# dylandreimerink/mimic

Hardware: AMD Instinct MI355X
Metric: Mpkts/s (device-resident, one XDP program over 64-1500B batches) (higher is better)
Workload: dtype u64; 1 GPU; cfg2: 1M x 64B xdp_md, 36-slot parse+hash DROP/PASS classifier, per-CPU array E=4 S=8; packets_per_gpu=1048576, vcpus_per_gpu=262144, schedule=interleaved, parallelism=dp1, batches_rotated=8, working_set_bytes=713031680, program_slots=36, engine=spread_own, batches_per_launch=8

## Files before the change

### mimic_amd/csrc/engine.cpp

```cpp
#include <hip/hip_runtime.h>

#include <algorithm>
#include <atomic>
#include <cstdarg>
#include <cstdlib>
#include <cstdio>
#include <cstring>
#include <map>
#include <string>
#include <chrono>
#include <condition_variable>
#include <memory>
#include <mutex>
#include <thread>
#include <unordered_map>
#include <vector>

#include "../../include/mimic_amd.h"
#include "blkcache.h"
#include "layout.h"
#include "hashmap.h"
#include "jit.h"
#include "skb.h"

// ... 1835 lines not shown
            while (q > 1 && (P % q || 256u * q / P > rows)) q--;
            kp->own_q = q;
            own = ko.state > 0 && P % q == 0 && 256u * q / P <= rows && 256u * q / P >= 1u &&
                  mimic_jit_step_bound(ko.info, kp->max_tail_calls) <= kp->budget;
            spread = own;
        }
        if (!own && (knob == 1 || (knob != 0 && (uint64_t)b->n >= 8ull * cpu_lanes))) {
            if ((rc = spread_build(vm, false))) return rc;
            const JitKernel &ks = vm->kern[K_SPREAD];
            spread = ks.state > 0 && mimic_jit_step_bound(ks.info, kp->max_tail_calls) <= kp->budget;
            if (knob != 1 && !ks.info.spread_rows && cpu_lanes > 16384) spread = false;
        }
    }
    const bool cxk = jit && kp->cancel_any;
    if (cxk) {
        spread = own = false;
        if (!vm->kern[K_CX + ctx].state) {
            const std::vector<std::pair<uint32_t, uint32_t>> vc = percpu_slots(vm).vc;
            JitOpts o;
            o.ctx_kind = ctx;
            o.vc_slots = &vc;
            o.no_early_loads = !lane.info.early_loads;
            o.ctx_check = true;
            if ((rc = kern_build(vm, o, "", &vm->kern[K_CX + ctx]))) return rc;
        }
    }
    *out = KernChoice{proc_jit ? K_PROC : own ? K_OWN : spread ? K_SPREAD : cxk ? K_CX + (int)ctx : K_LANE + (int)ctx,
                      jit, spread, own};
    const JitKernel &k = vm->kern[out->form];
    if (proc_jit && (!k.fn || !k.info.proc_ok)) return fail(vm, MIMIC_EDEVICE, "process: no single-process JIT kernel (engine)");
    return 0;
}

static int run_xdp_impl(mimic_vm *vm, uint32_t prog_id, const mimic_xdp_batch *b, const mimic_xdp_results *res,
                        hipStream_t st_in, uint64_t first_index, const SkbRun *skb, const StepRun *step,
                        const CtxRun *cx, ManyRun *mr) {
    if (!vm || !b || !res) return MIMIC_EINVAL;
    if (prog_id >= vm->progs.size()) return fail(vm, MIMIC_EINVAL, "no program with id '%u' is loaded", prog_id);
    if (const int brc = xdp_batch_check(vm, b, -1)) return brc;
    if (skb && b->n > 0 && (!b->pkt_off || !b->pkt_len)) return fail(vm, MIMIC_EINVAL, "missing packet arrays");
    if (cx && cx->all && cx->per_packet) return fail(vm, MIMIC_EINVAL, "one context for the batch or one per packet, not both");
    if (cx && cx->all && !cx->all->pinned) return fail(vm, MIMIC_EDEVICE, "the context was made without a device");
    if (cx && cx->per_packet)
        for (uint32_t i = 0; i < b->n; i++)
            if (cx->per_packet[i] && !cx->per_packet[i]->pinned)
                return fail(vm, MIMIC_EDEVICE, "packet %u: the context was made without a device", i);
    if (!skb) {
        const int rc = skb_settle(vm);
        if (rc) return rc;
    }
    if (!skb && vm->skb_leaked)
        return fail(vm, MIMIC_ENOTSUP, "xdp_md batches after sk_buff batches are not supported (mimic_skb_release first)");
    const uint32_t ctx = skb ? CTX_SKB : CTX_XDP;
    hipSetDevice(vm->s.device);
    int rc = upload_tables(vm);
    if (!rc) rc = flush_host(vm);
    if (rc) return rc;
    hipStream_t st = st_in ? st_in : vm->stream;
    const uint32_t cpu_lanes = step ? 1u : (uint32_t)vm->s.vcpu_count;
    const bool proc_jit = step && step->jit;
    bool extra = false;
    if (!step && b->schedule == MIMIC_SCHED_EXPLICIT && b->cpu)
        for (uint32_t i = 0; i < b->n && !extra; i++) extra = b->cpu[i] == -1 || b->cpu[i] == vm->s.vcpus;
    const uint32_t lanes = cpu_lanes + (extra ? 2u : 0u);
    const uint32_t S = stack_size(vm);
    const PrivPlan pp = priv_plan(vm);
// ... 238 lines not shown
    }
    vm->last_exec = jit ? (own ? MIMIC_EXEC_SPREAD_OWN : spread ? MIMIC_EXEC_SPREAD : MIMIC_EXEC_JIT) : MIMIC_EXEC_INTERP;
    if (jit && ji.defer) {
        if (lanes > vm->defer_cap || !vm->d_defer_any) {
            hipStreamSynchronize(st);
            hipFree(vm->d_defer);
            vm->d_defer = nullptr;
            HIP_OK(vm, hipMalloc(&vm->d_defer, (uint64_t)plan * sizeof(DeferRec)));
            HIP_OK(vm, hipMemset(vm->d_defer, 0, (uint64_t)plan * sizeof(DeferRec)));
            vm->defer_cap = plan;
            if (!vm->d_defer_any) {
                HIP_OK(vm, hipMalloc(&vm->d_defer_any, 64));
                HIP_OK(vm, hipMemset(vm->d_defer_any, 0, 64));
            }
        }
        if (++vm->defer_epoch == 0) vm->defer_epoch = 1;
        kp.defer = vm->d_defer;
        kp.defer_any = vm->d_defer_any;
        kp.defer_epoch = vm->defer_epoch;
    }
    if (jit && ji.hash_combine) vm->comb_used = true;
    if (mr) {
        mr->used = jit && own && !ji.defer && mr->k >= 1 && mr->k <= MIMIC_MANY_MAX;
        if (mr->used) {
            kp.many_n = mr->k;
            for (uint32_t q = 0; q < mr->k; q++) {
                const mimic_xdp_batch &bq = mr->b[q];
                kp.many[q] = BatchRef{bq.pkt_data, bq.pkt_off, bq.pkt_len, mr->r[q].r0, mr->r[q].status, mr->r[q].steps,
                                      mr->r[q].err_pc,
                                      (bq.pkt_off ? 0u : bq.pkt_stride) | (uint64_t)(bq.pkt_len ? 0u : bq.pkt_len_all) << 32};
            }
        }
    }
    if (jit) {
        if (mimic_jit_launch(kern.fn, &kp, st))
            return fail(vm, MIMIC_EDEVICE, "launch: %s", hipGetErrorString(hipGetLastError()));
        if (ji.defer && mimic_launch_xdp_resume(&kp, st))
            return fail(vm, MIMIC_EDEVICE, "launch: %s", hipGetErrorString(hipGetLastError()));
    } else if (step) {
        if (mimic_launch_xdp(&kp, nullptr, st))
            return fail(vm, MIMIC_EDEVICE, "launch: %s", hipGetErrorString(hipGetLastError()));
    } else {
        const KParams *dkp = nullptr;
        const int slot = kp_slot(vm, kp, st, &dkp);
        if (slot < 0) return slot;
        if (mimic_launch_xdp(&kp, dkp, st))
            return fail(vm, MIMIC_EDEVICE, "launch: %s", hipGetErrorString(hipGetLastError()));
        HIP_OK(vm, hipEventRecord(vm->kp_ev[slot], st));
        vm->kp_used[slot] = true;
    }
    if (jit && ji.hash_chunk) {
        for (const HostMap &m : vm->maps) {
            if (!m.chunk) continue;
            const DMap dm = to_dmap(m);
            if (mimic_launch_hash_compact(vm->arena, &dm, st))
                return fail(vm, MIMIC_EDEVICE, "launch: %s", hipGetErrorString(hipGetLastError()));
        }
    }
    if (jit && kp.spread_part) {
        const DMap dm = to_dmap(vm->maps[ji.spread_map]);
        if (mimic_launch_spread_reduce(kp.spread_part, kp.lanes / 256u, kp.cpu_lanes, ji.spread_roww, ji.spread_n,
                                       vm->arena + dm.dev_off + (uint64_t)kp.vcpu_begin * dm.dev_stride, dm.dev_stride, st))
            return fail(vm, MIMIC_EDEVICE, "launch: %s", hipGetErrorString(hipGetLastError()));
    }
    if (kp.cancel_any) {
        auto mark = [&](mimic_ctx *c) -> int {
            std::lock_guard<std::mutex> lk(c->mu);
            std::vector<hipEvent_t> keep;
// ... 935 lines not shown
```

### mimic_amd/csrc/jit.cpp

```cpp
#include <hip/hip_runtime.h>
#include <hip/hiprtc.h>

#include <algorithm>
#include <cinttypes>
#include <cstdarg>
#include <cstdio>
#include <cstring>
#include <cstdlib>
#include <unistd.h>
#include <map>
#include <mutex>
#include <set>
#include <string>
#include <vector>

#include "../../include/mimic_amd.h"
#include "layout.h"
#include "jit.h"

namespace {

#include "jit_headers.inc"

struct Emitter {
// ... 390 lines not shown
        E.line("      srow_ = lam_ >= lam0_ ? lam_ - lam0_ : lam_ + kp.cpu_lanes - lam0_;");
        E.line("      sbase_ = SM_.backing_addr + (uint32_t)L.cpu * SM_.addr_period; }");
        emit_xdp_load();
        emit_process_start("P + L.M + 1", "    uint64_t r10 = kp.static_next + kp.frame_size;");
        emit_entry_dispatch("kp.entry_prog");
        emit_programs();
        emit_result_stores("kq_", nullptr);
        emit_loop_close();
        E.line("#if SPREAD_ROWS");
        E.line("  __syncthreads();");
        E.line("  if (kp.spread_part && kp.cpu_lanes == SPREAD_ROWS) {");
        E.line("    spread_t *pt_ = (spread_t *)kp.spread_part + (size_t)blockIdx.x * (SPREAD_ROWS * SPREAD_ROWW);");
        E.line("    for (uint32_t w_ = threadIdx.x; w_ < SPREAD_ROWS * SPREAD_ROWW; w_ += 256u) {");
        E.line("      const uint32_t r_ = w_ / SPREAD_ROWW, q_ = w_ - r_ * SPREAD_ROWW;");
        E.line("      const uint32_t lr_ = lam0_ + r_ < SPREAD_ROWS ? lam0_ + r_ : lam0_ + r_ - SPREAD_ROWS;");
        E.line("      pt_[lr_ * SPREAD_ROWW + q_] = sacc_[w_];");
        E.line("    }");
        E.line("  } else");
        E.line("  for (uint32_t w_ = threadIdx.x; w_ < SPREAD_ROWS * SPREAD_ROWW; w_ += 256u) {");
        E.line("    const spread_t v_ = sacc_[w_];");
        E.line("    if (!v_) continue;");
        E.line("    const uint32_t r_ = w_ / SPREAD_ROWW, q_ = w_ - r_ * SPREAD_ROWW;");
        E.line("    const uint32_t lr_ = lam0_ + r_ < kp.cpu_lanes ? lam0_ + r_ : lam0_ + r_ - kp.cpu_lanes;");
        E.line("    spread_t *d_ = (spread_t *)(kp.arena + SM_.dev_off + (size_t)(kp.vcpu_begin + lr_) * SM_.dev_stride) + q_;");
        E.line("    __hip_atomic_fetch_add((GAS spread_t *)d_, v_, __ATOMIC_RELAXED, __HIP_MEMORY_SCOPE_AGENT);");
        E.line("  }");
        E.line("#endif");
        emit_kernel_close();
    }

    void emit_owned() {
        emit_kernel_open("0xffffffffu");
        emit_lane_open();
        E.line("  const uint32_t oP_ = kp.per_lane, oQ_ = kp.own_q, oS_ = oP_ / oQ_, oR_ = 256u / oS_;");
        E.line("  const uint32_t orow_ = threadIdx.x %% oR_, oj_ = threadIdx.x / oR_, olane_ = blockIdx.x * oR_ + orow_;");
        E.line("  const uint32_t osh_ = olane_ >= kp.sched_shift ? olane_ - kp.sched_shift : olane_ + kp.cpu_lanes - kp.sched_shift;");
        E.line("#define OWN_IDX_I(k_) ((oj_ < oS_ && olane_ < kp.cpu_lanes && (uint64_t)(oj_ + (k_) * oS_) * kp.cpu_lanes + osh_ < kp.n) ? (uint32_t)((uint64_t)(oj_ + (k_) * oS_) * kp.cpu_lanes + osh_) : NO_PKT)");
        E.line("#define OWN_IDX_C(k_) ((threadIdx.x + 256u * (k_) < oR_ * oP_ && (uint64_t)blockIdx.x * oR_ * oP_ + threadIdx.x + 256u * (k_) < kp.n) ? (uint32_t)((uint64_t)blockIdx.x * oR_ * oP_ + threadIdx.x + 256u * (k_)) : NO_PKT)");
        E.line("#define OWN_IDX(k_) (kp.sched == SCHED_CHUNKED ? OWN_IDX_C(k_) : OWN_IDX_I(k_))");
        E.line("  const uint32_t oi_ = OWN_IDX(0u);");
        E.line("  const bool ochk_ = kp.sched == SCHED_CHUNKED;");
        E.line("  const uint64_t ostr64_ = ochk_ ? 256ull : (uint64_t)oS_ * kp.cpu_lanes;");
        E.line("  const uint64_t oend_ = (uint64_t)blockIdx.x * oR_ * oP_ + (uint32_t)(oR_ * oP_);");
        E.line("  uint32_t ofl_ = __builtin_amdgcn_readfirstlane((kp.headroom_arr || kp.tailroom_arr || kp.ingress_arr || kp.rxq_arr || kp.egress_arr ? 1u : 0u) | (kp.headroom | kp.tailroom ? 2u : 0u));");
        E.line("  uint32_t ocpu_ = kp.vcpu_begin + olane_, oep_ = kp.entry_prog, or10_ = kp.static_next + kp.frame_size;");
        E.line("  uint32_t ostr_ = ostr64_ < 0xffffffffull ? (uint32_t)ostr64_ : 0xffffffffu;");
        E.line("  uint32_t olim_ = ochk_ && oend_ < kp.n ? (uint32_t)oend_ : kp.n;");
        E.line("  asm volatile(\"\" : \"+s\"(ostr_), \"+s\"(olim_), \"+s\"(ofl_), \"+s\"(oep_), \"+s\"(or10_));");
        E.line("  asm volatile(\"\" : \"+v\"(ocpu_));");
        E.line("  uint32_t oin_ = (uint32_t)kp.ingress, orx_ = (uint32_t)kp.rxq, oeg_ = (uint32_t)kp.egress;");
        E.line("  asm volatile(\"\" : \"+s\"(oin_), \"+s\"(orx_), \"+s\"(oeg_));");
        Emitter head;
        std::swap(head, E);
        E.line("  const DMap SM_ = cget(kp.maps, SPREAD_MAP);");
        E.line("  __shared__ spread_t sacc_[SPREAD_ROWS * SPREAD_ROWW];");
        E.line("  for (uint32_t w_ = threadIdx.x; w_ < SPREAD_ROWS * SPREAD_ROWW; w_ += 256u) sacc_[w_] = 0;");
        E.line("  __shared__ BatchRef obr_[MIMIC_MANY_MAX];");
        E.line("  if (threadIdx.x < (kp.many_n ? kp.many_n : 1u)) obr_[threadIdx.x] = kp.many_n ? cget(kp.many, threadIdx.x) : BatchRef{kp.pkt_data, kp.pkt_off, kp.pkt_len, kp.r0, kp.status, kp.steps, kp.err_pc, kp.pkt_stride | (uint64_t)kp.pkt_len_all << 32};");
        E.line("  __syncthreads();");
        E.line("  uint32_t srow_ = orow_, sbase_ = 0;");
        E.line("  const bool ofw_ = threadIdx.x < oR_ * SPREAD_ROWW && blockIdx.x * oR_ + threadIdx.x / SPREAD_ROWW < kp.cpu_lanes;");
        E.line("  GAS spread_t *const ofd_ = (GAS spread_t *)(kp.arena + SM_.dev_off + (size_t)(kp.vcpu_begin + blockIdx.x * oR_ + threadIdx.x / SPREAD_ROWW) * SM_.dev_stride) + threadIdx.x %% SPREAD_ROWW;");
        E.line("  const spread_t ofv_ = ofw_ ? *ofd_ : (spread_t)0;");
        emit_locals();
        if (pf) E.line("  uint64_t noff_ = 0, poff_ = 0; uint32_t nlen_ = 0, plen_ = 0;");
        E.line("  const uint32_t nb_ = kp.many_n ? kp.many_n : 1u;");
        E.line("  bool bpre_ = false;   // this batch's first descriptor came with the previous batch's last packet");
        E.line("  for (uint32_t bt_ = 0; bt_ < nb_; bt_++) {");
        E.line("  const BatchRef br_ = kp.many_n ? cget(kp.many, bt_) : BatchRef{kp.pkt_data, kp.pkt_off, kp.pkt_len, kp.r0, kp.status, kp.steps, kp.err_pc, kp.pkt_stride | (uint64_t)kp.pkt_len_all << 32};");
        E.line("  uint32_t cstr_ = (uint32_t)br_.compact, clen_ = (uint32_t)(br_.compact >> 32);");
        E.line("  asm volatile(\"\" : \"+v\"(cstr_), \"+v\"(clen_));");
        E.line("  ofl_ = (ofl_ & 3u) | (br_.pkt_off ? 0u : 4u) | (br_.pkt_len ? 0u : 8u);");
        if (pf) {
            E.line("  if (oi_ != NO_PKT) {");
            E.line("    if (!bpre_) { pkt_off_pf(!(ofl_ & 4u), br_.pkt_off, oi_, noff_); pkt_len_pf(!(ofl_ & 8u), br_.pkt_len, oi_, nlen_); }");
            E.line("    poff_ = pkt_off_take(!(ofl_ & 4u), noff_, cstr_, oi_); plen_ = pkt_len_take(!(ofl_ & 8u), nlen_, clen_);");
            E.line("  }");
            E.line("  bpre_ = false;");
        }
        E.line("  uint32_t oni_ = oi_;   // the thread's next packet");
        E.line("  for (uint32_t j = 0; j < oQ_; j++) {   // the thread's packets of its lane, in order");
        E.line("    const uint32_t i = oni_;");
        E.line("    if (i == NO_PKT) break;");
        E.line("    oni_ = NO_PKT;");
        E.line("    if (j + 1u < oQ_) { const uint64_t x_ = (uint64_t)i + ostr_; if (x_ < olim_) oni_ = (uint32_t)x_; }");
        if (pf) {
            E.line("    uint32_t cf_ = ofl_; asm volatile(\"\" : \"+s\"(cf_));");
            E.line("    const uint64_t *po_ = nullptr; const uint32_t *pl_ = nullptr;");
            E.line("    if (j + 1u < oQ_) { if (oni_ != NO_PKT && (cf_ & 12u) != 12u) { po_ = (cf_ & 4u) ? (const uint64_t *)&kp : br_.pkt_off + oni_; pl_ = (cf_ & 8u) ? (const uint32_t *)&kp : br_.pkt_len + oni_; } }");
            E.line("    else if (bt_ + 1u < nb_ && oi_ != NO_PKT) { const BatchRef &nx_ = obr_[bt_ + 1u];");
            E.line("      if (nx_.pkt_off || nx_.pkt_len) { po_ = nx_.pkt_off ? nx_.pkt_off + oi_ : (const uint64_t *)&kp; pl_ = nx_.pkt_len ? nx_.pkt_len + oi_ : (const uint32_t *)&kp; }");
            E.line("      bpre_ = true; }");
            E.line("    if (po_) { pkt_off_pf(true, po_, 0u, noff_); pkt_len_pf(true, pl_, 0u, nlen_); }");
        }
        emit_kq();
        E.line("    { const uint32_t ol_ = ochk_ ? i / oP_ : olane_;");
        E.line("      srow_ = ol_ - blockIdx.x * oR_;");
        E.line("      L.cpu = (int32_t)(ocpu_ - olane_ + ol_);");
        E.line("      sbase_ = SM_.backing_addr + (uint32_t)L.cpu * SM_.addr_period; }");
        E.line("    uint32_t H = 0u, T = 0u;");
        E.line("    L.ingress = oin_; L.rxq = orx_; L.egress = oeg_;");
        E.line("    if (ofl_ & 3u) {");
        E.line("      H = kq_.headroom_arr ? ld_nt(kq_.headroom_arr + i) : kq_.headroom;");
        E.line("      T = kq_.tailroom_arr ? ld_nt(kq_.tailroom_arr + i) : kq_.tailroom;");
        E.line("      if (kq_.ingress_arr) L.ingress = (uint32_t)ld_nt(kq_.ingress_arr + i);");
        E.line("      if (kq_.rxq_arr) L.rxq = (uint32_t)ld_nt(kq_.rxq_arr + i);");
        E.line("      if (kq_.egress_arr) L.egress = (uint32_t)ld_nt(kq_.egress_arr + i);");
        E.line("    }");
        emit_xdp_extent("br_.pkt_data", "pkt_len_at(!(ofl_ & 8u), br_.pkt_len, clen_, i)",
                        "pkt_off_at(!(ofl_ & 4u), br_.pkt_off, cstr_, i)", "if (ofl_ & 3u)");
        emit_process_start("P + L.M + 1", "    uint32_t lr10_ = or10_; asm volatile(\"\" : \"+s\"(lr10_));\n    uint64_t r10 = lr10_;");
        emit_entry_dispatch("oep_");
        emit_programs();
        if (pf) E.line("    { uint32_t ct_ = ofl_; asm volatile(\"\" : \"+s\"(ct_)); poff_ = pkt_off_take(!(ct_ & 4u), noff_, cstr_, oni_); plen_ = pkt_len_take(!(ct_ & 8u), nlen_, clen_); asm volatile(\"\" : \"+v\"(poff_), \"+v\"(plen_)); }");
        emit_result_stores("lb_", "    const BatchRef &lb_ = obr_[bt_];");
        emit_loop_close();
        E.line("  }   // batches");
        E.line("  __syncthreads();");
        E.line("  if (ofw_ && sacc_[threadIdx.x]) *ofd_ = ofv_ + sacc_[threadIdx.x];");
        E.line("  for (uint32_t w_ = threadIdx.x + 256u; w_ < oR_ * SPREAD_ROWW; w_ += 256u) {   // rows past 256 words");
        E.line("    const spread_t v_ = sacc_[w_];");
        E.line("    if (!v_) continue;");
        E.line("    const uint32_t r_ = w_ / SPREAD_ROWW, q_ = w_ - r_ * SPREAD_ROWW;");
        E.line("    GAS spread_t *d_ = (GAS spread_t *)(kp.arena + SM_.dev_off + (size_t)(kp.vcpu_begin + blockIdx.x * oR_ + r_) * SM_.dev_stride) + q_;");
        E.line("    *d_ += v_;");
        E.line("  }");
        emit_kernel_close();
        for (uint32_t s : own_k) head.line("  uint64_t hk%u_ = cget(kp.insns, %uu).k; asm volatile(\"\" : \"+s\"(hk%u_));", s, s, s);
        for (uint32_t s : own_h) head.line("  uint32_t hh%u_ = AUX_MAPHINT(cget(kp.insns, %uu).aux); asm volatile(\"\" : \"+s\"(hh%u_));", s, s, s);
        if (own_k.empty() && own_h.empty()) head.s += '\n';
        E.s = head.s + E.s;
    }

    void emit_kernel_open(const char *chunk_lanes) {
        E.line("extern \"C\" __global__ __launch_bounds__(256) %svoid mimic_jit_kernel(const KParams kp_arg_) {",
               waves_attr > 0 ? ("__attribute__((amdgpu_waves_per_eu(" + std::to_string(waves_attr) + "))) ").c_str() : "");
        E.line("  (void)kp_arg_;   // the first (only) kernel argument: at offset 0 of the kernarg segment");
        E.line("  const KParams __attribute__((address_space(4))) *kp4_ = (const KParams __attribute__((address_space(4))) *)__builtin_amdgcn_kernarg_segment_ptr();");
        E.line("  asm volatile(\"\" : \"+s\"(kp4_));");
        E.line("  const KParams *kpp = (const KParams *)kp4_;");
        E.line("  const KParams &kp = *kpp;");
        E.line("  const uint32_t g = blockIdx.x * blockDim.x + threadIdx.x;");
        if (hash_chunk) E.line("  h_chunk_init(%s);   // (its waves: those the early return below keeps)", chunk_lanes);
        if (hash_combine) E.line("  h_comb_init();   // before any thread of the block can leave");
    }
    void emit_lane_open() {
        if (skb_lds) E.line("  __shared__ uint64_t srec_[%uu * 256u];", kSrecQ);
        E.line("  Lane L;");
        E.line("  Spill sp_;");
        if (census) {
            E.line("  uint32_t coldn_ = 0;");
            E.line("#define COLD_CALL_K(k_, call_, pc_) do { coldn_ += 1u << (k_); COLD_CALL(call_, pc_); } while (0)");
        }
        E.line("  L.lane = g;");
    }
    void emit_vc_open() {
        if (vc_lds) {
            E.line("  __shared__ uint32_t lvc_[(%uu / 4u + 2u) * 256u];", vc_rb);
            E.line("  uint32_t *const lvt_ = lvc_ + threadIdx.x;");
            E.line("  constexpr uint32_t vcb_ = %uu;   // the row's bytes", vc_rb);
            E.line("  uint32_t vcv_ = 0u, vcd_ = 0u, vclo_ = 0u; uint8_t *vcp_ = nullptr;");
        } else {
            E.line("  uint64_t vc0_ = 0, vc1_ = 0, vc2_ = 0, vc3_ = 0; uint32_t vcv_ = 0u, vcd_ = 0u, vclo_ = 0u, vcb_ = 0u; uint8_t *vcp_ = nullptr;");
        }
        E.line("  { const uint32_t mh_ = AUX_MAPHINT(cget(kp.insns, %uu).aux);", vc_slot);
        if (vc_lds) E.line("    if (mh_) lvc_open(kp, cget(kp.maps, mh_ - 1u), L.cpu, vcb_, vcp_, vclo_, vcv_, lvt_); }");
        else E.line("    if (mh_) vc_open(kp, cget(kp.maps, mh_ - 1u), L.cpu, vcp_, vclo_, vcb_, vcv_, vc0_, vc1_, vc2_, vc3_); }");
    }
    void emit_locals() {
        E.line("  uint32_t ex_begin = 0, ex_count = 0;");
        E.line("  if (kp.sched == SCHED_EXPLICIT) { ex_begin = *gp(kp.sched_start + g); ex_count = *gp(kp.sched_start + g + 1) - ex_begin; }");
        E.line("  uint64_t lane_steps = 0;");
        E.line("  const uint32_t P = kp.static_next + kp.stack_size + 1;");
        if (ctx == CTX_SKB) E.line("  const uint32_t SK_ = P;   // the sk_buff entry (skb.h)");
        E.line("  uint32_t ga_ = 0;   // the address of the current memory access");
        if (ret_dispatch && any_local) E.line("  uint32_t ret_ = 0;   // the slot a popped frame returns to (R<p>_)");
        for (auto &f : fwd_store) E.line("  uint32_t fwd%u_%u_ = 0;   // value of the stack store at P%u slot %u", f.first, f.second, f.first, f.second);
        for (auto &u : spec_use)
            E.line("  %s sp%u_%u_ = 0;   // packet load of P%u slot %u, issued early", u.second == 8 ? "uint64_t" : "uint32_t",
                   u.first.first, u.first.second, u.first.first, u.first.second);
        if (!spec_use.empty()) E.line("  uint32_t spv_ = 1;   // 0 once a store through R10 left the stack: early values void");
    }
    void emit_pf_first(const char *next, const char *ok) {
        E.line("  uint64_t noff_ = 0; uint32_t nlen_ = 0;");
        E.line("  { const uint32_t n_ = %s; if (%s) pkt_desc_pf(kp, n_, noff_, nlen_); }", next, ok);
    }
    void emit_pf_next(const char *next, const char *ok) {
        E.line("    const uint64_t poff_ = pkt_off_take(kp, noff_, i); const uint32_t plen_ = pkt_len_take(kp, nlen_);");
        E.line("    { const uint32_t n_ = %s; if (%s) pkt_desc_pf(kp, n_, noff_, nlen_); }", next, ok);
    }
    void emit_kq() { E.line("    const KParams &kq_ = kp;"); }
    void emit_skb_load() {
        E.line("    uint64_t r1 = 0;");
        if (skb_lds)
            E.line("    const int ls_ = skb_load_lds(kp, L, i, r1, srec_ + %uu * threadIdx.x);", kSrecQ);
        else
            E.line("    const int ls_ = skb_load(kp, L, i, r1);");
    }
    void emit_xdp_load() {
        E.line("    const uint32_t H = kq_.headroom_arr ? ld_nt(kq_.headroom_arr + i) : kq_.headroom;");
        E.line("    const uint32_t T = kq_.tailroom_arr ? ld_nt(kq_.tailroom_arr + i) : kq_.tailroom;");
        emit_xdp_extent("kq_.pkt_data", "pkt_len_at(kq_, i)", "pkt_off_at(kq_, i)", nullptr);
        E.line("    L.ingress = (uint32_t)(kq_.ingress_arr ? ld_nt(kq_.ingress_arr + i) : kq_.ingress);");
        E.line("    L.rxq = (uint32_t)(kq_.rxq_arr ? ld_nt(kq_.rxq_arr + i) : kq_.rxq);");
        E.line("    L.egress = (uint32_t)(kq_.egress_arr ? ld_nt(kq_.egress_arr + i) : kq_.egress);");
    }
// ... 1406 lines not shown

std::string mimic_jit_source(const std::vector<DProg> &progs, const std::vector<DInsn> &all, const JitOpts &o,
                             JitInfo *info) {
    std::vector<ProgView> v;
    for (size_t p = 0; p < progs.size(); p++) v.push_back(ProgView{(uint32_t)p, progs[p].n, progs[p].base, all.data() + progs[p].base});
    Gen g(v, o.ctx_kind);
    if (o.vc_slots)
        for (auto &v : *o.vc_slots)
            if (v.second > 0 && v.second <= MIMIC_VC_MAX_ROW && !(v.second & 7)) g.vc_ok[v.first] = v.second;
    if (o.no_early_loads) g.speculate = 0;
    g.spread_req = o.spread;
    static const bool ctx_env = getenv("MIMIC_JIT_CTXCHECK") && getenv("MIMIC_JIT_CTXCHECK")[0] == '1';
    g.ctx_check = o.ctx_check || ctx_env;
    g.proc = o.proc;
    if (o.proc) g.inc_knob = false;
    std::string src = g.source();
    if (info) {
        info->checks_budget = g.careful_copies;
        info->max_n = g.max_n;
        info->tail_calls = g.has_tail();
        info->early_loads = g.has_early_loads();
        info->cold_inline = g.cold_inline;
        info->defer = g.defer_mode;
        info->spread = g.spread_on;
        info->spread_own = g.spread_own;
        info->hash_combine = g.hash_combine;
        info->hash_chunk = g.hash_chunk;
        info->proc = o.proc;
        info->proc_ok = o.proc && o.ctx_kind == CTX_XDP && !g.careful_copies && !g.defer_mode && !g.spread_on && !g.census;
        info->spread_map = g.spread_map;
        info->spread_n = g.spread_n;
        info->spread_roww = g.spread_n ? g.spread_row / g.spread_n : 0;
        info->spread_rows = g.spread_on && o.spread ? o.spread->lds_rows : 0;
    }
    return src;
}

uint64_t mimic_jit_step_bound(const JitInfo &info, uint32_t max_tail_calls) {
    if (info.checks_budget) return 0;
    return (info.tail_calls ? (uint64_t)max_tail_calls + 1 : 1) * ((uint64_t)info.max_n + 1);
}

int mimic_jit_compile(int device, const std::string &src, hipFunction_t *fn, std::string *log) {
    std::lock_guard<std::mutex> lk(g_mu);
    const CacheKey key{device, src};
    auto it = g_cache.find(key);
    if (it != g_cache.end()) {
        *fn = it->second;
        return 0;
    }
    std::vector<char> code;
    if (build_code(src, code, log)) return -1;
    hipModule_t mod;
    hipError_t e = hipModuleLoadData(&mod, code.data());
    if (e != hipSuccess) {
        *log = std::string("hipModuleLoadData: ") + hipGetErrorString(e);
        return -1;
    }
    e = hipModuleGetFunction(fn, mod, "mimic_jit_kernel");
    if (e != hipSuccess) {
        *log = std::string("hipModuleGetFunction: ") + hipGetErrorString(e);
        return -1;
    }
    g_cache[key] = *fn;
    return 0;
}

int mimic_jit_build_code(const std::string &src, std::vector<char> &code, std::string *log) {
    return build_code(src, code, log);
}

int mimic_jit_prebuild_source(const std::string &src, std::string *log) {
    std::vector<char> code;
    return build_code(src, code, log);
}

int mimic_jit_launch(hipFunction_t fn, const KParams *kp, hipStream_t st) {
    const uint32_t blocks = (kp->lanes + 255) / 256;
    if (blocks == 0) return 0;
    void *args[] = {(void *)kp};
    return hipModuleLaunchKernel(fn, blocks, 1, 1, 256, 1, 1, 0, st, args, nullptr) == hipSuccess ? 0 : -1;
}

int mimic_jit_check_source(const std::string &src, std::string *log, size_t *code_size) {
    setenv("AMD_COMGR_CACHE", "0", 0);
    hiprtcProgram prog;
    if (hiprtcCreateProgram(&prog, src.c_str(), "mimic_jit.hip", kJitHeaderCount, kJitHeaderSrc, kJitHeaderNames) !=
        HIPRTC_SUCCESS)
        return -1;
    const hiprtcResult rc = hiprtcCompileProgram(prog, kNOpts, kOpts);
    size_t ls = 0;
    hiprtcGetProgramLogSize(prog, &ls);
    std::string lg(ls + 1, '\0');
    if (ls) hiprtcGetProgramLog(prog, &lg[0]);
    *log = lg;
    if (code_size) hiprtcGetCodeSize(prog, code_size);
    hiprtcDestroyProgram(&prog);
    return rc == HIPRTC_SUCCESS ? 0 : -1;
}
```

### mimic_amd/csrc/jit.h

```cpp
#pragma once
#include <hip/hip_runtime.h>

#include <map>
#include <string>
#include <vector>

#include "layout.h"

struct JitInfo {
    bool checks_budget;
    uint32_t max_n;
    bool tail_calls;
    bool early_loads;
    bool cold_inline;
    bool defer;
    bool spread;
    bool spread_own;
    bool hash_combine;
    bool hash_chunk;
    bool proc, proc_ok;
    uint32_t spread_map, spread_n, spread_roww, spread_rows;
};
struct SpreadReq {
    std::map<uint32_t, uint32_t> slot_map;
    std::map<uint32_t, std::pair<uint32_t, uint32_t>> shape;
    uint32_t lds_rows = 0;
    uint32_t ppb = 1024;
    bool own = false;
};
#define MIMIC_VC_MAX_ROW 128u
struct JitOpts {
    uint32_t ctx_kind = CTX_XDP;
    const std::vector<std::pair<uint32_t, uint32_t>> *vc_slots = nullptr;
    bool no_early_loads = false;
    const SpreadReq *spread = nullptr;
    bool ctx_check = false;
    bool proc = false;
};
std::string mimic_jit_source(const std::vector<DProg> &progs, const std::vector<DInsn> &all, const JitOpts &o,
                             JitInfo *info);
uint64_t mimic_jit_step_bound(const JitInfo &info, uint32_t max_tail_calls);
int mimic_jit_compile(int device, const std::string &src, hipFunction_t *fn, std::string *log);
int mimic_jit_launch(hipFunction_t fn, const KParams *kp, hipStream_t st);
int mimic_jit_check_source(const std::string &src, std::string *log, size_t *code_size);
int mimic_jit_build_code(const std::string &src, std::vector<char> &code, std::string *log);
int mimic_jit_prebuild_source(const std::string &src, std::string *log);
```

### mimic_amd/csrc/layout.h

```cpp
#pragma once
#include <stdint.h>
#if defined(__HIPCC__) || defined(__HIP__) || defined(__HIPCC_RTC__)
#define HHD_LAYOUT static __host__ __device__ inline
#else
#define HHD_LAYOUT static inline
#endif

#define MIMIC_MAX_FRAMES 32u
#define MIMIC_DEFAULT_BUDGET (1ull << 22)
#define MIMIC_MEM_START 0x10000u
#define MIMIC_PC_BITS 24u
#define MIMIC_XDP_MD_SIZE 24u
#define MIMIC_FRAME_QWORDS 5u

enum SegKind : uint32_t {
    SEG_PLAIN = 1,
    SEG_ARRAY_OBJ = 2,
    SEG_MAP_OBJ = 3,
    SEG_PROG = 4,
    SEG_PERCPU_ARRAY = 5,
    SEG_PERCPU_VALUES = 6,
};

enum MapFamily : uint32_t { FAM_ARRAY = 1, FAM_PERCPU_ARRAY = 2, FAM_HASH = 3, FAM_PERCPU_HASH = 4 };
// ... 81 lines not shown
    H_LDABS = 14,
};
#define AUX_H(a) ((a) & 0xffu)
#define AUX_FALL_OK (1u << 8)
#define AUX_JT_OK (1u << 9)
#define AUX_JT_NEG (1u << 10)
#define AUX_W32 (1u << 11)
#define AUX_X (1u << 12)
#define AUX_ARG(a) (((a) >> 16) & 0xffu)
#define AUX_SZ(a) ((a) >> 24)
#define AUX_MAPHINT(a) ((a) >> 16)
struct DInsn {
    uint32_t w;
    uint32_t aux;
    uint64_t k;
};

enum Sched : uint32_t { SCHED_CHUNKED = 0, SCHED_INTERLEAVED = 1, SCHED_EXPLICIT = 2 };

enum CtxKind : uint32_t { CTX_XDP = 0, CTX_SKB = 1 };
struct SkbRec;

#define MIMIC_MANY_MAX 8u
struct BatchRef {
    uint8_t *pkt_data;
    const uint64_t *pkt_off;
    const uint32_t *pkt_len;
    uint64_t *r0;
    uint8_t *status;
    uint32_t *steps;
    int32_t *err_pc;
    uint64_t compact;
};

struct KParams {
    const DInsn *insns;
    const DProg *progs;
    const Seg *segs;
    const DMap *maps;
    uint8_t *arena;
    uint32_t nprogs, nsegs, nmaps, entry_prog;
    uint32_t static_next;
    uint32_t stack_size;
    uint32_t frame_size;
    uint32_t chunk_shift;
    uint32_t max_tail_calls;
    uint32_t total_vcpus;
    uint32_t vcpu_begin;
    uint32_t lanes;
    uint32_t priv_lanes;
    uint8_t *priv;
    uint32_t priv_xdp_q;
    uint32_t priv_frame_q;
    uint32_t priv_key_q;
    uint32_t cpu_lanes;
    uint64_t budget;
    uint32_t n;
    uint32_t sched;
    uint32_t per_lane;
    uint32_t sched_shift;
    uint8_t *pkt_data;
    const uint64_t *pkt_off;
    const uint32_t *pkt_len;
    const uint32_t *headroom_arr;
    const uint32_t *tailroom_arr;
    const int32_t *ingress_arr;
// ... 9 lines not shown
    uint32_t *steps;
    int32_t *err_pc;
    uint64_t *lane_steps;
    uint32_t ctx_kind;
    uint32_t skb_ifindex;
    SkbRec *skb_rec;
    const uint64_t *skb_prefix;
    const uint64_t *skb_base;
    struct StepState *step;
    uint32_t hash_pop_only;
    uint32_t hash_ro;
    struct DeferRec *defer;
    uint32_t *defer_any;
    uint32_t defer_epoch;
    uint32_t pkt_stride;
    uint32_t *spread_bad;
    const void *skb_custom;
    const uint64_t *skb_drv;
    void *spread_part;
    const uint32_t *cancel;
    const uint32_t *const *cancel_pp;
    uint32_t cancel_any;
    uint32_t own_q;
    uint32_t many_n;
    uint32_t pkt_len_all;
    struct BatchRef many[MIMIC_MANY_MAX];
    const uint8_t *step_img;
    uint8_t *step_dst;
    uint32_t step_img_n;
    uint32_t step_ins_n;
    uint32_t *skb_rooms_state;
};
static_assert(sizeof(KParams) == 968, "KParams: the kernarg layout of every JIT kernel");
static_assert(__builtin_offsetof(KParams, pkt_stride) == 356 && __builtin_offsetof(KParams, spread_bad) == 360,
              "KParams: the fields around the once reserved word keep their offsets");
static_assert(__builtin_offsetof(KParams, pkt_len_all) + 4 == __builtin_offsetof(KParams, many),
              "KParams: pkt_len_all fills the padding ahead of many[]");

struct DeferRec {
    uint64_t r[11];
    int32_t pc;
    uint32_t prog;
    uint32_t steps;
    uint32_t j;
    uint64_t lane_steps;
    uint64_t sm0, sm1;
    uint32_t xdp_dirty, nframes, tailcalls;
    uint32_t flag;
};

struct StepState {
    uint64_t r[11];
    int32_t pc;
    uint32_t prog;
    uint32_t steps;
    int32_t status;
    uint32_t started;
    uint32_t finished;
    int32_t cpu;
    uint32_t gen;
    uint8_t lane[256];
};
```

Before: 70740 Mpkts/s.

## Pass a precomputed OwnHead kernarg to the owned kernel and burst-load its header

Adds a second kernel argument (OwnHead) that the host fills with derived per-launch values: own_s/own_rows, r10, packet address, flags, spread-map row base/stride, and the hot instruction immediates and map hints. The owned kernel then reads these with a few scalar loads at a fixed kernarg offset, replacing divisions, DMap/insn table loads and per-batch BatchRef construction. It also adds a fast path for compact (stride/len-all) batches and prefetches the next batch's ref. The aim is a shorter kernel prologue and lower scalar-load latency, at the cost of a larger kernarg and a layout that other code must keep in sync.

```diff
diff --git a/mimic_amd/csrc/engine.cpp b/mimic_amd/csrc/engine.cpp
--- a/mimic_amd/csrc/engine.cpp
+++ b/mimic_amd/csrc/engine.cpp
@@ -1891,6 +1891,39 @@
     return 0;
 }
 
+static void own_head_fill(const mimic_vm *vm, const JitInfo &ji, KParams *kp, OwnHead *head) {
+    if (!kp->many_n)
+        kp->many[0] = BatchRef{kp->pkt_data, kp->pkt_off, kp->pkt_len, kp->r0, kp->status, kp->steps, kp->err_pc,
+                               kp->pkt_stride | (uint64_t)kp->pkt_len_all << 32};
+    OwnHead h{};
+    h.n = kp->n;
+    h.cpu_lanes = kp->cpu_lanes;
+    h.sched = kp->sched;
+    h.sched_shift = kp->sched_shift;
+    h.per_lane = kp->per_lane;
+    h.own_q = kp->own_q;
+    h.own_s = kp->per_lane / kp->own_q;
+    h.own_rows = 256u / h.own_s;
+    h.nb = kp->many_n ? kp->many_n : 1u;
+    h.vcpu_begin = kp->vcpu_begin;
+    h.entry_prog = kp->entry_prog;
+    h.r10 = kp->static_next + kp->frame_size;
+    h.pkt_addr = kp->static_next + kp->stack_size + 1;
+    h.flags = (kp->headroom_arr || kp->tailroom_arr || kp->ingress_arr || kp->rxq_arr || kp->egress_arr ? OWN_F_ARRAYS : 0u) |
+              (kp->headroom | kp->tailroom ? OWN_F_ROOMS : 0u);
+    h.ingress = (uint32_t)kp->ingress;
+    h.rxq = (uint32_t)kp->rxq;
+    h.egress = (uint32_t)kp->egress;
+    const DMap dm = to_dmap(vm->maps[ji.spread_map]);
+    h.sm_rows = kp->arena + dm.dev_off;
+    h.sm_stride = dm.dev_stride;
+    h.sm_backing_addr = dm.backing_addr;
+    h.sm_addr_period = dm.addr_period;
+    for (uint32_t k = 0; k < ji.own_hk_n; k++) h.hk[k] = vm->h_all[ji.own_hk[k]].k;
+    for (uint32_t k = 0; k < ji.own_hh_n; k++) h.hh[k] = AUX_MAPHINT(vm->h_all[ji.own_hh[k]].aux);
+    *head = h;
+}
+
 static int run_xdp_impl(mimic_vm *vm, uint32_t prog_id, const mimic_xdp_batch *b, const mimic_xdp_results *res,
                         hipStream_t st_in, uint64_t first_index, const SkbRun *skb, const StepRun *step,
                         const CtxRun *cx, ManyRun *mr) {
@@ -2195,8 +2228,10 @@
             }
         }
     }
+    OwnHead head{};
+    if (jit && own) own_head_fill(vm, ji, &kp, &head);
     if (jit) {
-        if (mimic_jit_launch(kern.fn, &kp, st))
+        if (mimic_jit_launch(kern.fn, &kp, own ? &head : nullptr, st))
             return fail(vm, MIMIC_EDEVICE, "launch: %s", hipGetErrorString(hipGetLastError()));
         if (ji.defer && mimic_launch_xdp_resume(&kp, st))
             return fail(vm, MIMIC_EDEVICE, "launch: %s", hipGetErrorString(hipGetLastError()));
diff --git a/mimic_amd/csrc/jit.cpp b/mimic_amd/csrc/jit.cpp
--- a/mimic_amd/csrc/jit.cpp
+++ b/mimic_amd/csrc/jit.cpp
@@ -446,49 +446,54 @@
     void emit_owned() {
         emit_kernel_open("0xffffffffu");
         emit_lane_open();
-        E.line("  const uint32_t oP_ = kp.per_lane, oQ_ = kp.own_q, oS_ = oP_ / oQ_, oR_ = 256u / oS_;");
+        Emitter open;
+        std::swap(open, E);
+        E.line("  const uint32_t oP_ = hd_.per_lane, oQ_ = hd_.own_q, oS_ = hd_.own_s, oR_ = hd_.own_rows;");
         E.line("  const uint32_t orow_ = threadIdx.x %% oR_, oj_ = threadIdx.x / oR_, olane_ = blockIdx.x * oR_ + orow_;");
-        E.line("  const uint32_t osh_ = olane_ >= kp.sched_shift ? olane_ - kp.sched_shift : olane_ + kp.cpu_lanes - kp.sched_shift;");
-        E.line("#define OWN_IDX_I(k_) ((oj_ < oS_ && olane_ < kp.cpu_lanes && (uint64_t)(oj_ + (k_) * oS_) * kp.cpu_lanes + osh_ < kp.n) ? (uint32_t)((uint64_t)(oj_ + (k_) * oS_) * kp.cpu_lanes + osh_) : NO_PKT)");
-        E.line("#define OWN_IDX_C(k_) ((threadIdx.x + 256u * (k_) < oR_ * oP_ && (uint64_t)blockIdx.x * oR_ * oP_ + threadIdx.x + 256u * (k_) < kp.n) ? (uint32_t)((uint64_t)blockIdx.x * oR_ * oP_ + threadIdx.x + 256u * (k_)) : NO_PKT)");
-        E.line("#define OWN_IDX(k_) (kp.sched == SCHED_CHUNKED ? OWN_IDX_C(k_) : OWN_IDX_I(k_))");
+        E.line("  const uint32_t osh_ = olane_ >= hd_.sched_shift ? olane_ - hd_.sched_shift : olane_ + hd_.cpu_lanes - hd_.sched_shift;");
+        E.line("#define OWN_IDX_I(k_) ((oj_ < oS_ && olane_ < hd_.cpu_lanes && (uint64_t)(oj_ + (k_) * oS_) * hd_.cpu_lanes + osh_ < hd_.n) ? (uint32_t)((uint64_t)(oj_ + (k_) * oS_) * hd_.cpu_lanes + osh_) : NO_PKT)");
+        E.line("#define OWN_IDX_C(k_) ((threadIdx.x + 256u * (k_) < oR_ * oP_ && (uint64_t)blockIdx.x * oR_ * oP_ + threadIdx.x + 256u * (k_) < hd_.n) ? (uint32_t)((uint64_t)blockIdx.x * oR_ * oP_ + threadIdx.x + 256u * (k_)) : NO_PKT)");
+        E.line("#define OWN_IDX(k_) (hd_.sched == SCHED_CHUNKED ? OWN_IDX_C(k_) : OWN_IDX_I(k_))");
         E.line("  const uint32_t oi_ = OWN_IDX(0u);");
-        E.line("  const bool ochk_ = kp.sched == SCHED_CHUNKED;");
-        E.line("  const uint64_t ostr64_ = ochk_ ? 256ull : (uint64_t)oS_ * kp.cpu_lanes;");
+        E.line("  const bool ochk_ = hd_.sched == SCHED_CHUNKED;");
+        E.line("  const uint64_t ostr64_ = ochk_ ? 256ull : (uint64_t)oS_ * hd_.cpu_lanes;");
         E.line("  const uint64_t oend_ = (uint64_t)blockIdx.x * oR_ * oP_ + (uint32_t)(oR_ * oP_);");
-        E.line("  uint32_t ofl_ = __builtin_amdgcn_readfirstlane((kp.headroom_arr || kp.tailroom_arr || kp.ingress_arr || kp.rxq_arr || kp.egress_arr ? 1u : 0u) | (kp.headroom | kp.tailroom ? 2u : 0u));");
-        E.line("  uint32_t ocpu_ = kp.vcpu_begin + olane_, oep_ = kp.entry_prog, or10_ = kp.static_next + kp.frame_size;");
+        E.line("  uint32_t ofl_ = hd_.flags & 3u;");
+        E.line("  uint32_t ocpu_ = hd_.vcpu_begin + olane_, oep_ = hd_.entry_prog, or10_ = hd_.r10;");
         E.line("  uint32_t ostr_ = ostr64_ < 0xffffffffull ? (uint32_t)ostr64_ : 0xffffffffu;");
-        E.line("  uint32_t olim_ = ochk_ && oend_ < kp.n ? (uint32_t)oend_ : kp.n;");
+        E.line("  uint32_t olim_ = ochk_ && oend_ < hd_.n ? (uint32_t)oend_ : hd_.n;");
         E.line("  asm volatile(\"\" : \"+s\"(ostr_), \"+s\"(olim_), \"+s\"(ofl_), \"+s\"(oep_), \"+s\"(or10_));");
         E.line("  asm volatile(\"\" : \"+v\"(ocpu_));");
-        E.line("  uint32_t oin_ = (uint32_t)kp.ingress, orx_ = (uint32_t)kp.rxq, oeg_ = (uint32_t)kp.egress;");
+        E.line("  uint32_t oin_ = hd_.ingress, orx_ = hd_.rxq, oeg_ = hd_.egress;");
         E.line("  asm volatile(\"\" : \"+s\"(oin_), \"+s\"(orx_), \"+s\"(oeg_));");
+        E.line("  uint32_t smb_ = hd_.sm_backing_addr, smp_ = hd_.sm_addr_period;");
+        E.line("  asm volatile(\"\" : \"+s\"(smb_), \"+s\"(smp_));");
         Emitter head;
         std::swap(head, E);
-        E.line("  const DMap SM_ = cget(kp.maps, SPREAD_MAP);");
         E.line("  __shared__ spread_t sacc_[SPREAD_ROWS * SPREAD_ROWW];");
         E.line("  for (uint32_t w_ = threadIdx.x; w_ < SPREAD_ROWS * SPREAD_ROWW; w_ += 256u) sacc_[w_] = 0;");
-        E.line("  __shared__ BatchRef obr_[MIMIC_MANY_MAX];");
-        E.line("  if (threadIdx.x < (kp.many_n ? kp.many_n : 1u)) obr_[threadIdx.x] = kp.many_n ? cget(kp.many, threadIdx.x) : BatchRef{kp.pkt_data, kp.pkt_off, kp.pkt_len, kp.r0, kp.status, kp.steps, kp.err_pc, kp.pkt_stride | (uint64_t)kp.pkt_len_all << 32};");
+        E.line("  if (threadIdx.x < MIMIC_MANY_MAX) obr_[threadIdx.x] = obv_;");
         E.line("  __syncthreads();");
         E.line("  uint32_t srow_ = orow_, sbase_ = 0;");
-        E.line("  const bool ofw_ = threadIdx.x < oR_ * SPREAD_ROWW && blockIdx.x * oR_ + threadIdx.x / SPREAD_ROWW < kp.cpu_lanes;");
-        E.line("  GAS spread_t *const ofd_ = (GAS spread_t *)(kp.arena + SM_.dev_off + (size_t)(kp.vcpu_begin + blockIdx.x * oR_ + threadIdx.x / SPREAD_ROWW) * SM_.dev_stride) + threadIdx.x %% SPREAD_ROWW;");
+        E.line("  const bool ofw_ = threadIdx.x < oR_ * SPREAD_ROWW && blockIdx.x * oR_ + threadIdx.x / SPREAD_ROWW < hd_.cpu_lanes;");
+        E.line("  GAS spread_t *const ofd_ = (GAS spread_t *)(hd_.sm_rows + (size_t)(hd_.vcpu_begin + blockIdx.x * oR_ + threadIdx.x / SPREAD_ROWW) * hd_.sm_stride) + threadIdx.x %% SPREAD_ROWW;");
         E.line("  const spread_t ofv_ = ofw_ ? *ofd_ : (spread_t)0;");
-        emit_locals();
+        emit_locals("hd_.pkt_addr", false);
         if (pf) E.line("  uint64_t noff_ = 0, poff_ = 0; uint32_t nlen_ = 0, plen_ = 0;");
-        E.line("  const uint32_t nb_ = kp.many_n ? kp.many_n : 1u;");
+        E.line("  const uint32_t nb_ = hd_.nb;");
         E.line("  bool bpre_ = false;   // this batch's first descriptor came with the previous batch's last packet");
         E.line("  for (uint32_t bt_ = 0; bt_ < nb_; bt_++) {");
-        E.line("  const BatchRef br_ = kp.many_n ? cget(kp.many, bt_) : BatchRef{kp.pkt_data, kp.pkt_off, kp.pkt_len, kp.r0, kp.status, kp.steps, kp.err_pc, kp.pkt_stride | (uint64_t)kp.pkt_len_all << 32};");
         E.line("  uint32_t cstr_ = (uint32_t)br_.compact, clen_ = (uint32_t)(br_.compact >> 32);");
         E.line("  asm volatile(\"\" : \"+v\"(cstr_), \"+v\"(clen_));");
         E.line("  ofl_ = (ofl_ & 3u) | (br_.pkt_off ? 0u : 4u) | (br_.pkt_len ? 0u : 8u);");
         if (pf) {
             E.line("  if (oi_ != NO_PKT) {");
-            E.line("    if (!bpre_) { pkt_off_pf(!(ofl_ & 4u), br_.pkt_off, oi_, noff_); pkt_len_pf(!(ofl_ & 8u), br_.pkt_len, oi_, nlen_); }");
-            E.line("    poff_ = pkt_off_take(!(ofl_ & 4u), noff_, cstr_, oi_); plen_ = pkt_len_take(!(ofl_ & 8u), nlen_, clen_);");
+            E.line("    if ((ofl_ & 12u) == 12u) { poff_ = (uint64_t)oi_ * cstr_; plen_ = clen_; }");
+            E.line("    else {");
+            E.line("      if (!bpre_) { pkt_off_pf(!(ofl_ & 4u), br_.pkt_off, oi_, noff_); pkt_len_pf(!(ofl_ & 8u), br_.pkt_len, oi_, nlen_); }");
+            E.line("      poff_ = pkt_off_take(!(ofl_ & 4u), noff_, cstr_, oi_); plen_ = pkt_len_take(!(ofl_ & 8u), nlen_, clen_);");
+            E.line("      asm volatile(\"\" : \"+v\"(poff_), \"+v\"(plen_));");
+            E.line("    }");
             E.line("  }");
             E.line("  bpre_ = false;");
         }
@@ -511,7 +516,7 @@
         E.line("    { const uint32_t ol_ = ochk_ ? i / oP_ : olane_;");
         E.line("      srow_ = ol_ - blockIdx.x * oR_;");
         E.line("      L.cpu = (int32_t)(ocpu_ - olane_ + ol_);");
-        E.line("      sbase_ = SM_.backing_addr + (uint32_t)L.cpu * SM_.addr_period; }");
+        E.line("      sbase_ = smb_ + (uint32_t)L.cpu * smp_; }");
         E.line("    uint32_t H = 0u, T = 0u;");
         E.line("    L.ingress = oin_; L.rxq = orx_; L.egress = oeg_;");
         E.line("    if (ofl_ & 3u) {");
@@ -520,6 +525,7 @@
         E.line("      if (kq_.ingress_arr) L.ingress = (uint32_t)ld_nt(kq_.ingress_arr + i);");
         E.line("      if (kq_.rxq_arr) L.rxq = (uint32_t)ld_nt(kq_.rxq_arr + i);");
         E.line("      if (kq_.egress_arr) L.egress = (uint32_t)ld_nt(kq_.egress_arr + i);");
+        E.line("      asm volatile(\"\" : \"+v\"(H), \"+v\"(T));");
         E.line("    }");
         emit_xdp_extent("br_.pkt_data", "pkt_len_at(!(ofl_ & 8u), br_.pkt_len, clen_, i)",
                         "pkt_off_at(!(ofl_ & 4u), br_.pkt_off, cstr_, i)", "if (ofl_ & 3u)");
@@ -529,26 +535,74 @@
         if (pf) E.line("    { uint32_t ct_ = ofl_; asm volatile(\"\" : \"+s\"(ct_)); poff_ = pkt_off_take(!(ct_ & 4u), noff_, cstr_, oni_); plen_ = pkt_len_take(!(ct_ & 8u), nlen_, clen_); asm volatile(\"\" : \"+v\"(poff_), \"+v\"(plen_)); }");
         emit_result_stores("lb_", "    const BatchRef &lb_ = obr_[bt_];");
         emit_loop_close();
+        E.line("  if (bt_ + 1u < nb_) br_ = cget(kp.many, bt_ + 1u);");
         E.line("  }   // batches");
         E.line("  __syncthreads();");
         E.line("  if (ofw_ && sacc_[threadIdx.x]) *ofd_ = ofv_ + sacc_[threadIdx.x];");
-        E.line("  for (uint32_t w_ = threadIdx.x + 256u; w_ < oR_ * SPREAD_ROWW; w_ += 256u) {   // rows past 256 words");
+        E.line("  if (threadIdx.x + 256u < SPREAD_ROWS * SPREAD_ROWW) {");
+        E.line("  const OwnHead CONST_AS *hf_ = hp4_; asm volatile(\"\" : \"+s\"(hf_));");
+        E.line("  const uint32_t fR_ = hf_->own_rows, fvb_ = hf_->vcpu_begin;");
+        E.line("  uint8_t *const frows_ = hf_->sm_rows; const uint64_t fstr_ = hf_->sm_stride;");
+        E.line("  for (uint32_t w_ = threadIdx.x + 256u; w_ < fR_ * SPREAD_ROWW; w_ += 256u) {   // rows past 256 words");
         E.line("    const spread_t v_ = sacc_[w_];");
         E.line("    if (!v_) continue;");
         E.line("    const uint32_t r_ = w_ / SPREAD_ROWW, q_ = w_ - r_ * SPREAD_ROWW;");
-        E.line("    GAS spread_t *d_ = (GAS spread_t *)(kp.arena + SM_.dev_off + (size_t)(kp.vcpu_begin + blockIdx.x * oR_ + r_) * SM_.dev_stride) + q_;");
+        E.line("    GAS spread_t *d_ = (GAS spread_t *)(frows_ + (size_t)(fvb_ + blockIdx.x * fR_ + r_) * fstr_) + q_;");
         E.line("    *d_ += v_;");
         E.line("  }");
+        E.line("  }");
         emit_kernel_close();
-        for (uint32_t s : own_k) head.line("  uint64_t hk%u_ = cget(kp.insns, %uu).k; asm volatile(\"\" : \"+s\"(hk%u_));", s, s, s);
-        for (uint32_t s : own_h) head.line("  uint32_t hh%u_ = AUX_MAPHINT(cget(kp.insns, %uu).aux); asm volatile(\"\" : \"+s\"(hh%u_));", s, s, s);
-        if (own_k.empty() && own_h.empty()) head.s += '\n';
-        E.s = head.s + E.s;
-    }
+        std::string hdecl, hpin;
+        uint32_t nk = 0, nh = 0;
+        for (uint32_t s : own_k) {
+            if (nk < MIMIC_HEAD_K) {
+                hdecl += "  uint64_t hk" + std::to_string(s) + "_ = hp4_->hk[" + std::to_string(nk) + "];\n";
+                hpin += ", \"+s\"(hk" + std::to_string(s) + "_)";
+            } else head.line("  uint64_t hk%u_ = cget(kp.insns, %uu).k; asm volatile(\"\" : \"+s\"(hk%u_));", s, s, s);
+            nk++;
+        }
+        for (uint32_t s : own_h) {
+            if (nh < MIMIC_HEAD_H) {
+                hdecl += "  uint32_t hh" + std::to_string(s) + "_ = hp4_->hh[" + std::to_string(nh) + "];\n";
+                hpin += ", \"+s\"(hh" + std::to_string(s) + "_)";
+            } else head.line("  uint32_t hh%u_ = AUX_MAPHINT(cget(kp.insns, %uu).aux); asm volatile(\"\" : \"+s\"(hh%u_));", s, s, s);
+            nh++;
+        }
+        own_burst(open, hdecl, hpin);
+        E.s = open.s + head.s + E.s;
+    }
+    void own_burst(Emitter &o, const std::string &hdecl, const std::string &hpin) {
+        o.line("  __shared__ BatchRef obr_[MIMIC_MANY_MAX];");
+        o.line("  BatchRef obv_ = BatchRef{};");
+        o.line("  if (threadIdx.x < MIMIC_MANY_MAX) obv_ = cget(kp.many, threadIdx.x);");
+        o.line("  (void)hd_arg_;   // the second argument: in the kernarg segment behind KParams");
+        o.line("  const OwnHead CONST_AS *hp4_ = (const OwnHead CONST_AS *)((const char CONST_AS *)kp4_ + MIMIC_OWN_HEAD_OFF);");
+        o.line("  OwnHead hd_ = OwnHead{}; BatchRef br_ = BatchRef{};");
+        static const char *const w0[] = {"n", "cpu_lanes", "sched", "sched_shift", "per_lane", "own_q", "own_s", "own_rows", "nb",
+                                         "vcpu_begin", "entry_prog", "r10", "pkt_addr", "flags", "ingress", "rxq"};
+        static const char *const w1[] = {"sm_rows", "sm_stride", "sm_backing_addr", "sm_addr_period", "egress"};
+        static const char *const wb[] = {"pkt_data", "pkt_off", "pkt_len", "compact"};
+        std::string p0, p1;
+        for (const char *f : w0) { o.line("  hd_.%s = hp4_->%s;", f, f); p0 += std::string(p0.empty() ? "" : ", ") + "\"+s\"(hd_." + f + ")"; }
+        for (const char *f : w1) { o.line("  hd_.%s = hp4_->%s;", f, f); p1 += std::string(p1.empty() ? "" : ", ") + "\"+s\"(hd_." + f + ")"; }
+        for (const char *f : wb) { o.line("  br_.%s = kp4_->many[0].%s;", f, f); p1 += std::string(", \"+s\"(br_.") + f + ")"; }
+        o.s += hdecl;
+        o.line("  asm volatile(\"\" : %s, %s%s);", p0.c_str(), p1.c_str(), hpin.c_str());
+    }
+  public:
+    void own_slots(JitInfo *info) const {
+        info->own_hk_n = info->own_hh_n = 0;
+        for (uint32_t s : own_k)
+            if (info->own_hk_n < MIMIC_HEAD_K) info->own_hk[info->own_hk_n++] = s;
+        for (uint32_t s : own_h)
+            if (info->own_hh_n < MIMIC_HEAD_H) info->own_hh[info->own_hh_n++] = s;
+    }
+  private:
 
     void emit_kernel_open(const char *chunk_lanes) {
-        E.line("extern \"C\" __global__ __launch_bounds__(256) %svoid mimic_jit_kernel(const KParams kp_arg_) {",
-               waves_attr > 0 ? ("__attribute__((amdgpu_waves_per_eu(" + std::to_string(waves_attr) + "))) ").c_str() : "");
+        E.line("extern \"C\" __global__ __launch_bounds__(256) %svoid mimic_jit_kernel(const KParams kp_arg_%s) {",
+               waves_attr > 0 ? ("__attribute__((amdgpu_waves_per_eu(" + std::to_string(waves_attr) + "))) ").c_str() : "",
+               spread_own ? ", const OwnHead hd_arg_" : "");
         E.line("  (void)kp_arg_;   // the first (only) kernel argument: at offset 0 of the kernarg segment");
         E.line("  const KParams __attribute__((address_space(4))) *kp4_ = (const KParams __attribute__((address_space(4))) *)__builtin_amdgcn_kernarg_segment_ptr();");
         E.line("  asm volatile(\"\" : \"+s\"(kp4_));");
@@ -581,11 +635,11 @@
         if (vc_lds) E.line("    if (mh_) lvc_open(kp, cget(kp.maps, mh_ - 1u), L.cpu, vcb_, vcp_, vclo_, vcv_, lvt_); }");
         else E.line("    if (mh_) vc_open(kp, cget(kp.maps, mh_ - 1u), L.cpu, vcp_, vclo_, vcb_, vcv_, vc0_, vc1_, vc2_, vc3_); }");
     }
-    void emit_locals() {
+    void emit_locals(const char *pkt_addr = "kp.static_next + kp.stack_size + 1", bool explicit_sched = true) {
         E.line("  uint32_t ex_begin = 0, ex_count = 0;");
-        E.line("  if (kp.sched == SCHED_EXPLICIT) { ex_begin = *gp(kp.sched_start + g); ex_count = *gp(kp.sched_start + g + 1) - ex_begin; }");
+        if (explicit_sched) E.line("  if (kp.sched == SCHED_EXPLICIT) { ex_begin = *gp(kp.sched_start + g); ex_count = *gp(kp.sched_start + g + 1) - ex_begin; }");
         E.line("  uint64_t lane_steps = 0;");
-        E.line("  const uint32_t P = kp.static_next + kp.stack_size + 1;");
+        E.line("  const uint32_t P = %s;", pkt_addr);
         if (ctx == CTX_SKB) E.line("  const uint32_t SK_ = P;   // the sk_buff entry (skb.h)");
         E.line("  uint32_t ga_ = 0;   // the address of the current memory access");
         if (ret_dispatch && any_local) E.line("  uint32_t ret_ = 0;   // the slot a popped frame returns to (R<p>_)");
@@ -2058,6 +2112,7 @@
         info->spread_n = g.spread_n;
         info->spread_roww = g.spread_n ? g.spread_row / g.spread_n : 0;
         info->spread_rows = g.spread_on && o.spread ? o.spread->lds_rows : 0;
+        g.own_slots(info);
     }
     return src;
 }
@@ -2101,10 +2156,10 @@
     return build_code(src, code, log);
 }
 
-int mimic_jit_launch(hipFunction_t fn, const KParams *kp, hipStream_t st) {
+int mimic_jit_launch(hipFunction_t fn, const KParams *kp, const OwnHead *head, hipStream_t st) {
     const uint32_t blocks = (kp->lanes + 255) / 256;
     if (blocks == 0) return 0;
-    void *args[] = {(void *)kp};
+    void *args[] = {(void *)kp, (void *)head};
     return hipModuleLaunchKernel(fn, blocks, 1, 1, 256, 1, 1, 0, st, args, nullptr) == hipSuccess ? 0 : -1;
 }
 
diff --git a/mimic_amd/csrc/jit.h b/mimic_amd/csrc/jit.h
--- a/mimic_amd/csrc/jit.h
+++ b/mimic_amd/csrc/jit.h
@@ -20,6 +20,8 @@
     bool hash_chunk;
     bool proc, proc_ok;
     uint32_t spread_map, spread_n, spread_roww, spread_rows;
+    uint32_t own_hk_n, own_hh_n;
+    uint32_t own_hk[MIMIC_HEAD_K], own_hh[MIMIC_HEAD_H];
 };
 struct SpreadReq {
     std::map<uint32_t, uint32_t> slot_map;
@@ -41,7 +43,7 @@
                              JitInfo *info);
 uint64_t mimic_jit_step_bound(const JitInfo &info, uint32_t max_tail_calls);
 int mimic_jit_compile(int device, const std::string &src, hipFunction_t *fn, std::string *log);
-int mimic_jit_launch(hipFunction_t fn, const KParams *kp, hipStream_t st);
+int mimic_jit_launch(hipFunction_t fn, const KParams *kp, const OwnHead *head, hipStream_t st);
 int mimic_jit_check_source(const std::string &src, std::string *log, size_t *code_size);
 int mimic_jit_build_code(const std::string &src, std::vector<char> &code, std::string *log);
 int mimic_jit_prebuild_source(const std::string &src, std::string *log);
diff --git a/mimic_amd/csrc/layout.h b/mimic_amd/csrc/layout.h
--- a/mimic_amd/csrc/layout.h
+++ b/mimic_amd/csrc/layout.h
@@ -137,6 +137,29 @@
     int32_t *err_pc;
     uint64_t compact;
 };
+
+#define MIMIC_HEAD_K 8u
+#define MIMIC_HEAD_H 8u
+#define OWN_F_ARRAYS 1u
+#define OWN_F_ROOMS 2u
+struct alignas(64) OwnHead {
+    uint32_t n, cpu_lanes, sched, sched_shift;
+    uint32_t per_lane, own_q;
+    uint32_t own_s, own_rows;
+    uint32_t nb;
+    uint32_t vcpu_begin, entry_prog;
+    uint32_t r10;
+    uint32_t pkt_addr;
+    uint32_t flags;
+    uint32_t ingress, rxq;
+    uint8_t *sm_rows;
+    uint64_t sm_stride;
+    uint32_t sm_backing_addr, sm_addr_period;
+    uint32_t egress, pad;
+    uint32_t hh[MIMIC_HEAD_H];
+    uint64_t hk[MIMIC_HEAD_K];
+};
+static_assert(sizeof(OwnHead) == 192, "OwnHead: three 64-byte lines");
 
 struct KParams {
     const DInsn *insns;
@@ -212,6 +235,9 @@
     uint32_t *skb_rooms_state;
 };
 static_assert(sizeof(KParams) == 968, "KParams: the kernarg layout of every JIT kernel");
+#define MIMIC_OWN_HEAD_OFF 1024u
+static_assert(MIMIC_OWN_HEAD_OFF == (sizeof(KParams) + 63) / 64 * 64 && alignof(OwnHead) == 64,
+              "OwnHead: where the owned kernel reads it");
 static_assert(__builtin_offsetof(KParams, pkt_stride) == 356 && __builtin_offsetof(KParams, spread_bad) == 360,
               "KParams: the fields around the once reserved word keep their offsets");
 static_assert(__builtin_offsetof(KParams, pkt_len_all) + 4 == __builtin_offsetof(KParams, many),
```

New measurement: 69770 Mpkts/s. 0.986x the previous value.
